# nvpro-samples/vk_gltf_renderer

Hardware: AMD Instinct MI355X
Metric: Msamples/s (and ms/frame @ fixed spp) 1080p & 4K, 1/2/4/8 MI355X (higher is better)
Workload: dtype f32

## Files before the change

vk_gltf_renderer_amd/csrc/device/mi_pt_api.hip:

```cpp
#include <hip/hip_runtime.h>

#include <algorithm>
#include <chrono>
#include <cstdlib>
#include <cmath>
#include <cstdio>
#include <cstring>
#include <memory>
#include <string>
#include <vector>

#include "mi_pt.h"
#include "bvh_refit.h"
#include "dev_buf.h"
#include "material_patch.h"
#include "pt_build.h"
#include "pt_bvh.h"
#include "pt_deform.h"
#include "pt_kernels.h"

namespace {

thread_local std::string g_lastError;

int fail(int code, const std::string& msg)
{
  g_lastError = msg;
  return code;
}

#define HIP_TRY(x)                                                                                                       \
  do                                                                                                                    \
  {                                                                                                                     \
    hipError_t e_ = (x);                                                                                                \
    if(e_ != hipSuccess)                                                                                                \
      return fail(MI_PT_ERR_HIP, std::string(#x) + ": " + hipGetErrorString(e_));                                       \
  } while(0)

using pt::DevBuf;

enum TimedKernel { TK_GENERATE, TK_TRACE, TK_SORT, TK_SHADE, TK_SHADOW, TK_ACCUM, TK_PRIMARY, TK_SHADE_FIRST, TK_COUNT };

}

struct RunSwitches
{
  int    packetInterval = 1;
  int    sortMode       = 2;
  bool   noPacket       = false;
  bool   stateBySlot    = false;
  bool   traceSpans     = false;
  int    overlapUpTo    = 32;
  int    overlapMinTris = 200000;
  bool   noPlanes       = false;
  bool   noOpaqueTris   = false;
  bool   noQuads        = false;
  bool   shadowFarFirst = true;
  int    reinsert       = 16;
  int    reinsertUpdate = 0;
  int    reinsertRounds = 4;
  float  splitFactor    = 4.0f;
  int    splitMaxDepth  = 8;
  float  splitMinShare  = 0.1f;
  bool   collapseGreedy = false;
  bool   collapseBad    = false;
  bool   hostCollapse   = false;
  bool   coreTex        = true;
  bool   shadowDeposit  = true;
  int    maxItersDiag   = 0;
  int    failBuildAt    = 0;
  bool   candPoolSet    = false;
  size_t candPool       = 0;
  void   read()
  {
    auto flag = [](const char* n) { const char* e = getenv(n); return e != nullptr; };
    auto num  = [](const char* n, int d) { const char* e = getenv(n); return e ? atoi(e) : d; };
    packetInterval = num("MI_PT_PACKET_INTERVAL", 1);
    sortMode       = num("MI_PT_SORT", 2);
    noPacket       = flag("MI_PT_NO_PACKET");
    stateBySlot    = flag("MI_PT_STATE_BY_SLOT");
    traceSpans     = flag("MI_PT_TRACE_SPANS");
    overlapUpTo    = num("MI_PT_OVERLAP", 32);
    overlapMinTris = num("MI_PT_OVERLAP_MIN_TRIS", 200000);
    noPlanes       = flag("MI_PT_DIAG_NO_PLANES");
    noOpaqueTris   = flag("MI_PT_DIAG_NO_OPAQUE_TRIS");
    noQuads        = flag("MI_PT_DIAG_NO_QUADS");
    shadowFarFirst = num("MI_PT_SHADOW_FAR_FIRST", 1) != 0;
    reinsert       = std::max(0, num("MI_PT_REINSERT", 16));
    reinsertUpdate = std::max(0, num("MI_PT_REINSERT_UPDATE", 0));
    reinsertRounds = std::max(1, num("MI_PT_REINSERT_ROUNDS", 4));
    if(const char* e = getenv("MI_PT_SPLIT"))
      splitFactor = std::max(0.0f, float(atof(e)));
    if(const char* e = getenv("MI_PT_SPLIT_MIN_SHARE"))
      splitMinShare = std::max(0.0f, float(atof(e)));
    splitMaxDepth  = std::min(std::max(0, num("MI_PT_SPLIT_DEPTH", 8)), 10);
    if(const char* e = getenv("MI_PT_COLLAPSE"))
    {
      collapseGreedy = strcmp(e, "greedy") == 0;
      collapseBad    = !collapseGreedy && strcmp(e, "sah") != 0;
    }
    hostCollapse   = flag("MI_PT_HOST_COLLAPSE");
    maxItersDiag   = num("MI_PT_DIAG_MAX_ITERS", 0);
    coreTex        = num("MI_PT_CORE_TEX", 1) != 0;
    shadowDeposit  = num("MI_PT_SHADOW_DEPOSIT", 1) != 0;
    failBuildAt    = num("MI_PT_DIAG_FAIL_BUILD", 0);
    if(const char* e = getenv("MI_PT_DIAG_CAND_POOL"))
    {
      candPoolSet = true;
      candPool    = size_t(strtoull(e, nullptr, 10));
    }
  }
};

struct MiPt
{
  int device = 0;
  int numCUs = 256;
  RunSwitches sw;
  int accelBuilds = 0;
  int               frameQueueDepth = 1;
  int               pendingFrames   = 0;
  MiPathtraceParams pendingFirst{};
  void*             pendingStream   = nullptr;
  DevBuf<MiGltfShadeMaterial> materials;
  DevBuf<MiGltfTextureInfo>   texInfos;
  DevBuf<pt::DevTexRef>       texRefs;
  DevBuf<pt::DevCoreTex>      coreTex;
  DevBuf<MiGltfRenderNode>    nodes;
  DevBuf<pt::DevPrim>         prims;
  DevBuf<MiGltfLight>         lights;
  DevBuf<pt::DevTexture>      textures;
  DevBuf<uchar4>              texels;
  DevBuf<uint4>               texQuads;
  DevBuf<uint8_t>             geometry;
  DevBuf<uint8_t>             instFlags;
  DevBuf<float>               srgbLut;
  DevBuf<float4>              envPixels;
// ... 176 lines not shown
    return rc;
  if(!vertexMotionActive(pt))
    return MI_PT_OK;
  const size_t numPrims = pt->hostPrims.size();
  pt->vmPrevOffset.assign(numPrims, SIZE_MAX);
  size_t                bytes = 0;
  std::vector<uint32_t> ids;
  for(int id : pt->deformPrimIDs)
  {
    pt->vmPrevOffset[size_t(id)] = bytes;
    bytes += align16(size_t(pt->primVertices[size_t(id)]) * 12);
    pt->vmMaxVertices = std::max(pt->vmMaxVertices, pt->primVertices[size_t(id)]);
    ids.push_back(uint32_t(id));
  }
  HIP_TRY(pt->vmPrevPositions.alloc(std::max<size_t>(bytes, 16)));
  std::vector<pt::VertexMotionPrim> table(numPrims);
  for(size_t i = 0; i < numPrims; ++i)
  {
    pt::VertexMotionPrim& v = table[i];
    v.prevPositions = pt->vmPrevOffset[i] != SIZE_MAX ? reinterpret_cast<const float*>(pt->vmPrevPositions.ptr + pt->vmPrevOffset[i]) : nullptr;
    v.positions     = pt->hostPrims[i].positions;
    v.indices       = pt->hostPrims[i].indices;
    v.numTriangles  = i < pt->primTriangles.size() ? pt->primTriangles[i] : 0u;
    v.vertexCount   = pt->primVertices[i];
  }
  HIP_TRY(pt->vmPrims.upload(table.data(), table.size()));
  HIP_TRY(pt->vmDeformIDs.upload(ids.data(), ids.size()));
  pt::launchSnapshotPositions(pt->vmPrims.ptr, pt->vmDeformIDs.ptr, uint32_t(ids.size()), pt->vmMaxVertices, nullptr);
  HIP_TRY(hipGetLastError());
  HIP_TRY(hipDeviceSynchronize());
  return MI_PT_OK;
}

int allocPathResources(MiPt* pt, int frames)
{
  if(size_t(pt->numSlots) * size_t(frames) >= 0x7fffffffull)
    return fail(MI_PT_ERR_ARGUMENT, "too many path slots: reduce the frames in flight or the resolution");
  pt->framesCap          = frames;
  const size_t n         = std::max(size_t(pt->numSlots) * size_t(frames), size_t(1));
  HIP_TRY(pt->pathArrays.alloc(n));
  HIP_TRY(pt->firstHit.alloc(std::max(size_t(pt->numSlots), size_t(1))));
  pt->haveFirstHit = false;
  pt->optThroughput.release(); pt->optMisc.release(); pt->optMedium.release(); pt->optPixelSum.release(); pt->optGuides.release(); pt->optShadowAux2.release();
  pt::PathSoA& P = pt->paths;
  P              = pt::PathSoA{};
  P.radiance     = pt->pathArrays.ptr;
  P.firstHit     = pt->firstHit.ptr;
  if(int rc = allocFirstHitTri(pt))
    return rc;
  const size_t numChunks = (n + pt::QCHUNK - 1) / pt::QCHUNK;
  const size_t subCap    = ((numChunks + pt::NSUB - 1) / pt::NSUB + 1) * pt::QCHUNK;
  const size_t qsize     = subCap * pt::NSUB;
  if(qsize >= (size_t(1) << 31))
    return fail(MI_PT_ERR_ARGUMENT, "mi_pt_render_frames: " + std::to_string(frames) + " frames in flight x " + std::to_string(pt->numSlots)
                                        + " pixel slots exceed 2^31 path slots");
  HIP_TRY(pt->queueMem.alloc(qsize * 3 + pt::QC_COUNT));
  HIP_TRY(pt->queuePayload.alloc(qsize * 14));
  pt->queueCap = qsize;
  pt::RayQueue* qs[3] = {&pt->queues.active[0], &pt->queues.active[1], &pt->queues.shadow};
  for(int i = 0; i < 3; ++i)
    qs[i]->slot = pt->queueMem.ptr + qsize * size_t(i);
  for(int i = 0; i < 2; ++i)
  {
    qs[i]->org  = pt->queuePayload.ptr + qsize * size_t(5 * i + 0);
    qs[i]->dir  = pt->queuePayload.ptr + qsize * size_t(5 * i + 1);
    qs[i]->aux2 = pt->queuePayload.ptr + qsize * size_t(5 * i + 2);
    qs[i]->misc = pt->queuePayload.ptr + qsize * size_t(5 * i + 3);
    qs[i]->rad  = pt->queuePayload.ptr + qsize * size_t(5 * i + 4);
    qs[i]->aux  = pt->queuePayload.ptr + qsize * 10;
  }
  pt->queues.shadow.org  = pt->queuePayload.ptr + qsize * 11;
  pt->queues.shadow.dir  = pt->queuePayload.ptr + qsize * 12;
  pt->queues.shadow.aux  = pt->queuePayload.ptr + qsize * 13;
  pt->queues.shadow.aux2 = nullptr;
  pt->queues.shadow.misc = pt->queues.shadow.rad = nullptr;
  pt->queues.counters = pt->queueMem.ptr + 3 * qsize;
  pt->queues.subCap   = uint32_t(subCap);
  pt->queues.candPool = nullptr; pt->queues.candNext = nullptr; pt->queues.overflow = nullptr;
  pt->queues.candCap  = 0;
  size_t candCap = qsize * 2;
  if(pt->sw.candPoolSet)
    candCap = pt->sw.candPool;
  if(pt->hasTransmissive && pt->wide && candCap > 0)
  {
// ... 765 lines not shown
  }
  {
    std::string why;
    if(!materialSlotsInRange(sd->materials, sd->numMaterials, sd->numTextureInfos, why))
      return fail(MI_PT_ERR_ARGUMENT, "mi_pt_create: " + why);
  }
  for(int i = 0; i < sd->numRenderPrimitives; ++i)
  {
    const MiPtRenderPrimitive& p = sd->renderPrimitives[i];
    if(p.vertexCount > 0 && !p.positions)
      return fail(MI_PT_ERR_ARGUMENT, "mi_pt_create: render primitive " + std::to_string(i) + " has vertices but no positions");
    if(p.triangleCount > 0 && !p.indices)
      return fail(MI_PT_ERR_ARGUMENT, "mi_pt_create: render primitive " + std::to_string(i) + " has triangles but no indices");
    for(size_t k = 0, n = size_t(p.triangleCount) * 3; k < n; ++k)
      if(p.indices[k] >= p.vertexCount)
        return fail(MI_PT_ERR_ARGUMENT, "mi_pt_create: render primitive " + std::to_string(i) + " has a vertex index beyond its vertexCount");
  }

  static const bool buildTiming = getenv("MI_PT_BUILD_TIMING") != nullptr;
  auto              tPhase      = std::chrono::steady_clock::now();
  auto              phase       = [&](const char* what) {
    if(!buildTiming)
      return;
    (void)hipDeviceSynchronize();
    const auto now = std::chrono::steady_clock::now();
    fprintf(stderr, "[mi_pt build] %-28s %8.2f ms\n", what, std::chrono::duration<double, std::milli>(now - tPhase).count());
    tPhase = now;
  };

  std::unique_ptr<MiPt> pt(new MiPt());
  pt->sw.read();
  if(pt->sw.collapseBad)
    return fail(MI_PT_ERR_ARGUMENT, std::string("MI_PT_COLLAPSE=") + getenv("MI_PT_COLLAPSE") + " is neither \"sah\" nor \"greedy\"");
  pt->device          = device;
  pt->numCUs          = prop.multiProcessorCount > 0 ? prop.multiProcessorCount : 256;
  pt->collectCounters = options && options->collectCounters;

  HIP_TRY(pt->materials.upload(sd->materials, size_t(sd->numMaterials)));
  HIP_TRY(pt->texInfos.upload(sd->textureInfos, size_t(sd->numTextureInfos)));
  HIP_TRY(pt->nodes.upload(sd->renderNodes, size_t(sd->numRenderNodes)));
  HIP_TRY(pt->lights.upload(sd->lights, size_t(sd->numLights)));

  size_t geomBytes = 0;
  for(int i = 0; i < sd->numRenderPrimitives; ++i)
  {
    const MiPtRenderPrimitive& p = sd->renderPrimitives[i];
    geomBytes += align16(size_t(p.triangleCount) * 12);
    geomBytes += align16(size_t(p.vertexCount) * 12);
    if(p.normals) geomBytes += align16(size_t(p.vertexCount) * 12);
    if(p.colors) geomBytes += align16(size_t(p.vertexCount) * 4);
    if(p.tangents) geomBytes += align16(size_t(p.vertexCount) * 16);
    if(p.texCoords0) geomBytes += align16(size_t(p.vertexCount) * 8);
    if(p.texCoords1) geomBytes += align16(size_t(p.vertexCount) * 8);
    geomBytes += align16(size_t(p.vertexCount) * 48);
  }
  if(geomBytes / 16 >= (size_t(1) << 32))
    return fail(MI_PT_ERR_ARGUMENT, "the geometry pool exceeds 64 GiB");
  HIP_TRY(pt->geometry.alloc(std::max<size_t>(geomBytes, 16)));
  std::vector<uint8_t>     staging(std::max<size_t>(geomBytes, 16));
  std::vector<pt::DevPrim> devPrims(size_t(sd->numRenderPrimitives));
  {
    size_t off = 0;
    auto   put = [&](const void* src, size_t bytes) -> const uint8_t* {
      if(!src || bytes == 0)
        return nullptr;
      memcpy(staging.data() + off, src, bytes);
// ... 772 lines not shown
  c.fc.numFrames = numFrames;
  pt::divideMagic(uint32_t(std::max(numFrames, 2)), c.fc.framesMagic, c.fc.framesShift);
  c.fc.slotLayout = numFrames % 64 == 0 ? 1 : 0;
  c.fc.stateInQueue = (!pt->sw.stateBySlot && !(pt->frameInfo.flags & MI_SCENE_INFINITE_PLANE_SHADOW_CATCHER)) ? 1 : 0;
  const bool guides = (params->flags & MI_PT_USE_OPTIX_DENOISER) != 0;
  if(int rc = ensureOptionalPathArrays(pt, c.fc.stateInQueue == 0, params->numSamples > 1, guides, (pt->frameInfo.flags & MI_SCENE_INFINITE_PLANE_SHADOW_CATCHER) != 0))
    return rc;
  c.paths        = pt->paths;
  {
    const bool stateBySlot = c.fc.stateInQueue == 0, multiSample = params->numSamples > 1;
    if(!(stateBySlot || multiSample))
      c.paths.misc = nullptr;
    if(!stateBySlot)
      c.paths.throughput = nullptr;
    if(!multiSample)
      c.paths.pixelSum = nullptr;
  }
  pt->accumFrames   = float(params->totalSamples) / float(params->numSamples) + float(numFrames);
  if(guides && (params->totalSamples == 0 || pt->momentFrames == pt->accumFrames - float(numFrames)))
    pt->momentFrames = pt->accumFrames;
  else if(!guides || params->totalSamples == 0)
    pt->momentFrames = 0.0f;
  if(!guides)
  {
    c.paths.guideAlbedo = nullptr;
    c.paths.guideNormal = nullptr;
  }
  c.queues           = pt->queues;
  if(!(pt->frameInfo.flags & MI_SCENE_INFINITE_PLANE_SHADOW_CATCHER))
    c.queues.shadow.aux2 = nullptr;
  c.ownedTiles       = pt->ownedTiles.ptr;
  c.stats            = pt->stats.ptr;
  c.stream           = stream;
  c.persistentBlocks = unsigned(pt->numCUs) * 8u;
  c.hasAlpha         = pt->hasAlpha;
  c.hasAlphaClosest  = c.hasAlpha && pt->hasAlphaTest;
  c.visualization    = pt->frameInfo.visualization > MI_VIZ_RENDERED && pt->frameInfo.visualization < MI_VIZ_COUNT;
  if(pt->frameInfo.visualization == MI_VIZ_OPACITY_MICROMAP)
    c.hasAlphaClosest = false;
  c.hasTransmissive  = pt->hasTransmissive;
  c.simpleMaterials  = pt->simpleMaterials;
  c.wide             = pt->wide;
  c.collectCounters  = pt->collectCounters;
  c.shadowDeposit    = pt->sw.shadowDeposit;
  {
    c.sortMode = pt->sw.sortMode;
  }
  if(pt->sceneDevDirty)
  {
    HIP_TRY(hipDeviceSynchronize());
    HIP_TRY(pt->sceneDev.upload(&pt->scene, 1));
    pt->sceneDevDirty = false;
  }
  if(!pt->fcHost)
  {
    HIP_TRY(hipHostMalloc(reinterpret_cast<void**>(&pt->fcHost), sizeof(pt::FrameConsts) * MiPt::FC_RING, hipHostMallocDefault));
    HIP_TRY(pt->fcRing.alloc(MiPt::FC_RING));
    for(hipEvent_t& e : pt->fcDone)
      HIP_TRY(hipEventCreateWithFlags(&e, hipEventDisableTiming));
  }
  const unsigned fcSlot = pt->fcCursor++ % unsigned(MiPt::FC_RING);
  if(pt->fcCursor > unsigned(MiPt::FC_RING))
    HIP_TRY(hipEventSynchronize(pt->fcDone[fcSlot]));
  pt->fcHost[fcSlot] = c.fc;
  HIP_TRY(hipMemcpyAsync(pt->fcRing.ptr + fcSlot, pt->fcHost + fcSlot, sizeof(pt::FrameConsts), hipMemcpyHostToDevice, stream));
  c.sceneDev = pt->sceneDev.ptr;
  c.fcDev    = pt->fcRing.ptr + fcSlot;

  auto timedOn = [&](hipStream_t on, int kind, auto&& launch) {
    if(pt->timingEnabled)
    {
      hipEvent_t a = getEvent(pt, pt->evCursor), b = getEvent(pt, pt->evCursor);
      (void)hipEventRecord(a, on);
      launch();
      (void)hipEventRecord(b, on);
      pt->pendingSpans.push_back({kind, a, b});
    }
// ... 709 lines not shown
```

vk_gltf_renderer_amd/csrc/device/pt_kernels.h:

```cpp
#pragma once
#include <hip/hip_runtime.h>

#include "pt_scene.h"
#include "pt_temporal.h"

namespace pt {

struct LaunchCtx
{
  DevScene        scene;
  FrameConsts     fc;
  const DevScene*    sceneDev;
  const FrameConsts* fcDev;
  PathSoA         paths;
  Queues          queues;
  const uint32_t* ownedTiles;
  StatCounters*   stats;
  hipStream_t     stream;
  unsigned        persistentBlocks;
  bool            hasAlpha;
  bool            hasAlphaClosest;
  bool            hasTransmissive;
  bool            simpleMaterials;
  bool            wide;
  bool            collectCounters;
  bool            shadowDeposit;
  int             sortMode;
  bool            visualization;
};

void launchBuildShadeRecords(const DevScene& scene, uint32_t numTris, DevShadeTri* out, hipStream_t s);
void launchBuildAlphaRecords(const DevScene& scene, uint32_t numTris, DevAlphaTri* out, hipStream_t s);
void launchPatchMaterials(const DevScene& scene, const uint8_t* instFlags, const uint8_t* dirty, DevTri* tris, DevAlphaTri* alphaTris, DevShadeTri* shadeTris,
                          uint32_t numTris, hipStream_t s);
void dumpTraceProfile();
void launchBvh8Planes(const uint4* nodes, uint32_t numNodes, float* planes, hipStream_t s);
void launchTextureQuads(const uchar4* texels, uint4* quads, uint32_t offset, int width, int height, int wrapS, int wrapT, hipStream_t s);
void launchResetCounters(const Queues& Q, hipStream_t s);
void launchSkyPrecomp(const MiSkyPhysicalParameters& sky, SkyPrecomp* out, hipStream_t stream);
void launchGenerate(const LaunchCtx& c, int sampleIndex);
void launchTraceClosest(const LaunchCtx& c, int cur);
void launchTracePrimary(const LaunchCtx& c, int sampleIndex);
void launchShade(const LaunchCtx& c, int cur, bool first);
void launchTraceShadow(const LaunchCtx& c, int nxt);
void launchFlushSurvivors(const LaunchCtx& c, int cur);
void launchFinishSample(const LaunchCtx& c, int sampleIndex, float4* accum, float* depth, float4* albedo, float4* normal);
void launchSelection(const LaunchCtx& c, uint32_t* selection);
void launchQueryRays(const DevScene& scene, bool wide, bool any, const MiPtRay* rays, uint32_t numRays, MiPtRayHit* hits, hipStream_t s);
void launchPickRays(const DevScene& scene, const FrameConsts& fc, bool wide, const float2* xy, uint32_t numRays, MiPtRayHit* hits, hipStream_t s);

void launchAtrous(const float4* in, float4* out, const float4* albedo, const float4* normal, int width, int height, int step, float sigmaColor,
                  float sigmaNormal, float sigmaAlbedo, hipStream_t s);

const float4* launchSvgf(const float4* color, const float4* albedo, const float4* normal, const float* depth, float4* bufA, float4* bufB, int width, int height,
                         int iterations, float frames, float sigmaLuminance, float sigmaNormal, float sigmaDepth, hipStream_t s);

const float4* launchSvgfFilter(float4* in, float4* other, const float4* color, const float4* albedo, const float4* normal, const float* depth, int width,
                               int height, int iterations, float sigmaLuminance, float sigmaNormal, float sigmaDepth, hipStream_t s);

// ... 13 lines not shown
```

vk_gltf_renderer_amd/csrc/device/pt_kernels.hip:

```cpp
#include <hip/hip_runtime.h>
#include <hip/hip_fp16.h>

#ifndef MI_PT_EXACT_FP
#define PT_FAST_SHADING_MATH 1
#endif
#include "pt_kernels.h"
#include "pt_shading.h"
#include "pt_bvh.h"
#include "pt_bvh8.h"
#include "pt_camera.h"
#include "pt_packet.h"
#include "pt_feed.h"
#include "pt_visualize.h"

namespace pt {

namespace {

constexpr int TRACE_BLOCK = 1024;
#ifndef NODE_CACHE_EXTRA
#define NODE_CACHE_EXTRA 0
#endif
constexpr int NODE_CACHE  = 712 + NODE_CACHE_EXTRA;
constexpr int NODE_CACHE_ALPHA = 504 + NODE_CACHE_EXTRA;
constexpr int SEL_BLOCK   = 256;
#ifndef TRACE_MIN_WAVES
#define TRACE_MIN_WAVES 1
#endif
constexpr int SHADE_BLOCK = 256;
constexpr uint32_t SORT_ROUNDS   = 4;
constexpr uint32_t SORT_WINDOW   = SORT_ROUNDS * SHADE_BLOCK;
constexpr uint32_t SORT_SEGMENTS = SORT_ROUNDS * (SHADE_BLOCK / 64);
constexpr int      SORT_BINS     = 32;
constexpr uint32_t SORT_BIN_MISS = 30;
constexpr uint32_t SORT_BIN_DEAD = 31;
#ifndef SHADE_SIMPLE_WAVES
#define SHADE_SIMPLE_WAVES 3
#endif

PT_DEV uint32_t laneId() { return __lane_id(); }

PT_DEV void queuePrefix(const uint32_t* counts, uint32_t* s_prefix)
{
  if(threadIdx.x < 64)
  {
// ... 33 lines not shown
    s_tmp[0] = 0;
    s_tmp[1] = 0;
  }
  __syncthreads();
  const unsigned long long maskN = __ballot(predNext), maskS = __ballot(predShadow);
  const uint32_t           lane  = laneId();
  uint32_t                 wbaseN = 0, wbaseS = 0;
  if(lane == 0)
  {
    if(maskN != 0ull)
      wbaseN = atomicAdd(&s_tmp[0], uint32_t(__popcll(maskN)));
    if(maskS != 0ull)
      wbaseS = atomicAdd(&s_tmp[1], uint32_t(__popcll(maskS)));
  }
  wbaseN = uint32_t(__shfl(int(wbaseN), 0));
  wbaseS = uint32_t(__shfl(int(wbaseS), 0));
  __syncthreads();
  if(threadIdx.x == 0)
  {
    const uint32_t     nN = s_tmp[0], nS = s_tmp[1];
    unsigned long long base = 0ull;
    if((nN | nS) != 0u)
      base = atomicAdd(reinterpret_cast<unsigned long long*>(pair), (static_cast<unsigned long long>(nS) << 32) | nN);
    s_tmp[2] = uint32_t(base);
    s_tmp[3] = uint32_t(base >> 32);
  }
  __syncthreads();
  const unsigned long long below = (1ull << lane) - 1ull;
  PushPos                  p;
  p.next   = sub * subCap + s_tmp[2] + wbaseN + uint32_t(__popcll(maskN & below));
  p.shadow = sub * subCap + s_tmp[3] + wbaseS + uint32_t(__popcll(maskS & below));
  return p;
}



PT_DEV bool slotToPixel(const FrameConsts& fc, const uint32_t* ownedTiles, uint32_t slot, int& px, int& py)
{
  const uint32_t tile  = ownedTiles[slot >> (2 * fc.tileShift)];
  const uint32_t w     = slot & ((1u << (2 * fc.tileShift)) - 1u);
  const uint32_t micro = w >> 6, lane = w & 63u;
  const uint32_t mshift = uint32_t(fc.tileShift) - 3u;
  px                   = int((tile & 0xffffu) + (micro & ((1u << mshift) - 1u)) * 8u + (lane & 7u));
  py                   = int((tile >> 16) + (micro >> mshift) * 8u + (lane >> 3));
  return px < fc.width && py < fc.height;
}


PT_DEV uint4 packMedium(f3 ext, f3 sc, float g)
{
  __half2 a = __floats2half2_rn(ext.x, ext.y), b = __floats2half2_rn(ext.z, sc.x), c = __floats2half2_rn(sc.y, sc.z), d = __floats2half2_rn(g, 0.0f);
  uint4   r;
  r.x = *reinterpret_cast<uint32_t*>(&a);
  r.y = *reinterpret_cast<uint32_t*>(&b);
  r.z = *reinterpret_cast<uint32_t*>(&c);
  r.w = *reinterpret_cast<uint32_t*>(&d);
  return r;
}
PT_DEV void unpackMedium(uint4 m, f3& ext, f3& sc, float& g)
{
  float2 a = __half22float2(*reinterpret_cast<__half2*>(&m.x)), b = __half22float2(*reinterpret_cast<__half2*>(&m.y));
  float2 c = __half22float2(*reinterpret_cast<__half2*>(&m.z)), d = __half22float2(*reinterpret_cast<__half2*>(&m.w));
  ext = mk3(a.x, a.y, b.x);
  sc  = mk3(b.y, c.x, c.y);
  g   = d.x;
}

struct CameraPath
// ... 1154 lines not shown
        if((G.bits >> 8) == 0u)
        {
          if(st2.sp == 0)
            break;
          G = st2.pop();
        }
        const uint32_t child = groupPopChild(G, octinv);
        if(G.bits >> 8)
          st2.push(G);
        uint32_t tBase, tMask;
        bvh8Visit(sc, r, bestT, octinv, child, G, tBase, tMask, nullptr, 0u);
        while(leafPending(tMask))
        {
          const int k = int(leafPop(tMask, 0u));
          testTri(int(tBase) + k);
        }
      }
    }
    else
    {
      LaneStack st;
      int       stackOverflow[BVH_STACK_PRIV];
      st.lds = s_stack; st.tid = int(threadIdx.x); st.stride = SEL_BLOCK; st.sp = 0; st.priv = stackOverflow;
      bvhWalk(sc, r, bestT, st, [&](int triIndex, float) -> float {
        testTri(triIndex);
        return bestT;
      });
    }
  }
  selection[size_t(py) * size_t(fc.width) + size_t(px)] = (bestRnode != 0xffffffffu) ? bestRnode + 1u : 0u;
}

template <bool COUNT, bool SIMPLE, bool FIRST>
__global__ void __launch_bounds__(SHADE_BLOCK, SIMPLE ? SHADE_SIMPLE_WAVES : 1) k_shade(const DevScene* __restrict__ scp, const FrameConsts* __restrict__ fcp, PathSoA P, Queues Q, int cur, int sortMode, StatCounters* stats)
{
  constexpr bool VIZ = false;
#include "pt_shade_body.h"
}
template <bool SIMPLE, bool FIRST>
__global__ void __launch_bounds__(SHADE_BLOCK, SIMPLE ? SHADE_SIMPLE_WAVES : 1) k_shade_viz(const DevScene* __restrict__ scp, const FrameConsts* __restrict__ fcp, PathSoA P, Queues Q, int cur, int sortMode, StatCounters* stats)
{
  constexpr bool COUNT = false, VIZ = true;
#include "pt_shade_body.h"
}

template <int MODE>
struct ShadowCfg
{
  static constexpr int BLOCK = MODE == 2 ? 256 : TRACE_BLOCK;
  static constexpr int CACHE = MODE == 2 ? 320 : (MODE == 1 ? NODE_CACHE_ALPHA : (MODE == 3 ? NODE_CACHE_ALPHA - 104 : NODE_CACHE));
};

PT_DEV void shadowDeposit(const PathSoA& P, const Queues& Q, int nxt, uint32_t slot, uint32_t qpos, bool catcherRay, f3 contrib, f3 total, bool occ,
                          float catcherDarken)
{
  if(!catcherRay)
  {
    if(!occ)
    {
      float4* const target = shadowTarget(P, Q, nxt, slot);
      float4        rad    = *target;
      rad.x += contrib.x * total.x;
      rad.y += contrib.y * total.y;
      rad.z += contrib.z * total.z;
      *target = rad;
    }
    return;
  }
  const float4 a2  = Q.shadow.aux2[qpos];
  const f3     sf  = occ ? mk3(0.0f) : total;
  float4       rad = P.radiance[slot];
  if(sf.x == 1.0f && sf.y == 1.0f && sf.z == 1.0f)
  {
// ... 939 lines not shown
  dim3           grid(batchSlots / 256u), block(256);
  const bool interval = c.fc.slotLayout == 1 && c.scene.packetInterval != 0 && c.scene.bvh8Planes != nullptr;
#define MI_LAUNCH_PRIMARY(A, C)                                                                                                                   \
  do                                                                                                                                              \
  {                                                                                                                                               \
    if(interval)                                                                                                                                  \
      hipLaunchKernelGGL((k_trace_primary<A, C, true>), grid, block, 0, c.stream, c.scene, c.fc, c.sceneDev, c.fcDev, c.paths, c.queues, c.ownedTiles, sampleIndex, batchSlots, c.stats);  \
    else                                                                                                                                          \
      hipLaunchKernelGGL((k_trace_primary<A, C, false>), grid, block, 0, c.stream, c.scene, c.fc, c.sceneDev, c.fcDev, c.paths, c.queues, c.ownedTiles, sampleIndex, batchSlots, c.stats); \
  } while(0)
  if(c.hasAlphaClosest)
  {
    if(c.collectCounters) MI_LAUNCH_PRIMARY(true, true); else MI_LAUNCH_PRIMARY(true, false);
  }
  else
  {
    if(c.collectCounters) MI_LAUNCH_PRIMARY(false, true); else MI_LAUNCH_PRIMARY(false, false);
  }
#undef MI_LAUNCH_PRIMARY
}
void launchTraceClosest(const LaunchCtx& c, int cur)
{
  if(c.wide)
    launchTraceClosestT<true>(c, cur);
  else
    launchTraceClosestT<false>(c, cur);
}
void launchShade(const LaunchCtx& c, int cur, bool first)
{
  dim3 grid(c.persistentBlocks), block(SHADE_BLOCK);
  if(c.visualization)
  {
#define MI_LAUNCH_SHADE_VIZ(S, F) \
  hipLaunchKernelGGL((k_shade_viz<S, F>), grid, block, 0, c.stream, c.sceneDev, c.fcDev, c.paths, c.queues, cur, (S ? 0 : c.sortMode), c.stats)
    if(c.simpleMaterials)
    {
      if(first) MI_LAUNCH_SHADE_VIZ(true, true); else MI_LAUNCH_SHADE_VIZ(true, false);
    }
    else
    {
      if(first) MI_LAUNCH_SHADE_VIZ(false, true); else MI_LAUNCH_SHADE_VIZ(false, false);
    }
#undef MI_LAUNCH_SHADE_VIZ
    return;
  }
#define MI_LAUNCH_SHADE(C, S, F) \
  hipLaunchKernelGGL((k_shade<C, S, F>), grid, block, 0, c.stream, c.sceneDev, c.fcDev, c.paths, c.queues, cur, (S ? 0 : c.sortMode), c.stats)
#define MI_LAUNCH_SHADE_F(C, S) do { if(first) MI_LAUNCH_SHADE(C, S, true); else MI_LAUNCH_SHADE(C, S, false); } while(0)
  if(c.simpleMaterials)
  {
    if(c.collectCounters) MI_LAUNCH_SHADE_F(true, true); else MI_LAUNCH_SHADE_F(false, true);
  }
  else
  {
    if(c.collectCounters) MI_LAUNCH_SHADE_F(true, false); else MI_LAUNCH_SHADE_F(false, false);
  }
#undef MI_LAUNCH_SHADE_F
#undef MI_LAUNCH_SHADE
}
void launchTraceShadow(const LaunchCtx& c, int nxt)
{
  if(c.wide)
    launchTraceShadowT<true>(c, nxt);
  else
    launchTraceShadowT<false>(c, nxt);
}
void launchFlushSurvivors(const LaunchCtx& c, int cur)
{
  hipLaunchKernelGGL(k_flush_survivors, dim3(c.persistentBlocks), dim3(256), 0, c.stream, c.paths, c.queues, cur);
}
void launchFinishSample(const LaunchCtx& c, int sampleIndex, float4* accum, float* depth, float4* albedo, float4* normal)
{
  unsigned grid = (unsigned(c.fc.numSlots) + 255u) / 256u;
  hipLaunchKernelGGL(k_finish_sample, dim3(grid), dim3(256), 0, c.stream, c.fc, c.sceneDev, c.fcDev, c.paths, c.ownedTiles, sampleIndex, accum, depth, albedo, normal);
}
void launchSelection(const LaunchCtx& c, uint32_t* selection)
{
  unsigned grid = (unsigned(c.fc.numSlots) + SEL_BLOCK - 1) / SEL_BLOCK;
  if(c.wide)
    hipLaunchKernelGGL(k_selection<true>, dim3(grid), dim3(SEL_BLOCK), 0, c.stream, c.scene, c.fc, c.ownedTiles, selection);
// ... 6 lines not shown
```

vk_gltf_renderer_amd/csrc/device/pt_shade_body.h:

```cpp
  const DevScene&    sc = uniformConst(*scp);
  const FrameConsts& fc = uniformConst(*fcp);
  const bool         stateInQueue = fc.stateInQueue != 0;
  __shared__ uint32_t s_prefix[NSUB + 1];
  __shared__ uint32_t s_push[4];
  __shared__ float    s_srgb[256];
#ifndef SHADE_NO_DEFERRED_MISS
  constexpr bool DEFER_MISS = !FIRST;
#else
  constexpr bool DEFER_MISS = false;
#endif
  __shared__ uint32_t s_missPos[DEFER_MISS ? 2 * SHADE_BLOCK : 1];
  __shared__ uint32_t s_missCount;
  const bool          deferMiss = DEFER_MISS && !hasFlag(fc.frameInfo.flags, MI_SCENE_USE_INFINITE_PLANE) && !hasFlag(fc.frameInfo.flags, MI_SCENE_USE_HDR_ENVIRONMENT);
  if(threadIdx.x == 0)
    s_missCount = 0;
  auto finishMisses = [&](bool all) {
    __syncthreads();
    const uint32_t n = s_missCount;
    if(n == 0u || (!all && n < uint32_t(SHADE_BLOCK)))
      return;
    const uint32_t take = min(n, uint32_t(SHADE_BLOCK)), base = n - take;
    uint32_t       pos = 0;
    if(threadIdx.x < take)
      pos = s_missPos[base + threadIdx.x];
    __syncthreads();
    if(threadIdx.x == 0)
      s_missCount = base;
    if(threadIdx.x < take)
    {
      const uint32_t slot  = Q.active[cur].slot[pos];
      const float4   d4    = Q.active[cur].dir[pos];
      const float4   misc4 = stateInQueue ? Q.active[cur].misc[pos] : P.misc[slot];
      const float4   tp4   = stateInQueue ? Q.active[cur].aux2[pos] : P.throughput[slot];
      const float4   rad4  = stateInQueue ? Q.active[cur].rad[pos] : P.radiance[slot];
      f3             radiance = xyz(rad4);
      f3             envColor;
      float          mis;
      missEnvironment(sc, fc, xyz(d4), tp4.w, envColor, mis);
      radiance += xyz(tp4) * mis * envColor;
      uint32_t flags = __float_as_uint(misc4.y) & (PF_INSIDE | PF_NOT_SOLID | (0xffu << PF_DEPTH_SHIFT) | (0xffu << PF_SCATTER_SHIFT));
      if(SIMPLE)
        flags &= ~uint32_t(PF_INSIDE);
      const bool solid = !(flags & PF_NOT_SOLID);
      P.radiance[slot] = make_float4(radiance.x, radiance.y, radiance.z, __uint_as_float(__float_as_uint(fmaxf(fabsf(rad4.w), 0.0f)) | (solid ? 0u : RADW_NOT_SOLID)));
      if(P.misc)
        P.misc[slot] = make_float4(misc4.x, __uint_as_float(flags), misc4.z, misc4.w);
    }
    __syncthreads();
  };
  constexpr bool CAN_SORT = !SIMPLE;
  __shared__ uint32_t s_order[CAN_SORT ? SORT_WINDOW : 1];
  __shared__ uint16_t s_segCount[CAN_SORT ? SORT_SEGMENTS : 1][SORT_BINS];
  __shared__ uint32_t s_binBase[SORT_BINS + 1];
  static_assert(SHADE_BLOCK == 256, "one table entry per thread");
  if(blockIdx.x == 0 && threadIdx.x < 8)
  {
    Q.counters[QC_HEADS_TRACE + threadIdx.x] = 0;
    Q.counters[QC_HEADS_SHADOW + threadIdx.x]   = 0;
    Q.counters[QC_HEADS_OVERFLOW + threadIdx.x] = 0;
    if(threadIdx.x == 0)
      Q.counters[QC_CAND_POOL] = Q.counters[QC_RESOLVE] = Q.counters[QC_OVERFLOW] = 0;
  }
  queuePrefix(&Q.counters[cur ? QC_PAIR1 : QC_PAIR0], s_prefix);
  const uint32_t count      = s_prefix[NSUB];
  const int      nxt        = cur ^ 1;
  constexpr uint32_t ROUNDS = CAN_SORT ? SORT_ROUNDS : 1u;
  constexpr uint32_t WINDOW = ROUNDS * SHADE_BLOCK;
  const uint32_t     numWindows = (count + WINDOW - 1) / WINDOW;
  if(blockIdx.x >= numWindows)
    return;
  s_srgb[threadIdx.x] = sc.srgbLut[threadIdx.x];
  __syncthreads();
  const uint32_t wave = threadIdx.x >> 6, lane = threadIdx.x & 63u;
  for(uint32_t win = blockIdx.x; win < numWindows; win += gridDim.x)
  {
    uint32_t live = min(WINDOW, count - win * WINDOW);
    if(CAN_SORT && sortMode != 0)
    {
    uint32_t myPos[SORT_ROUNDS], myBin[SORT_ROUNDS], myRank[SORT_ROUNDS];
    for(uint32_t t = threadIdx.x; t < SORT_SEGMENTS * SORT_BINS; t += SHADE_BLOCK)
      (&s_segCount[0][0])[t] = 0;
    __syncthreads();
#pragma unroll
    for(uint32_t k = 0; k < SORT_ROUNDS; ++k)
    {
      const uint32_t i = win * WINDOW + k * SHADE_BLOCK + threadIdx.x;
      uint32_t       bin = SORT_BIN_DEAD;
      myPos[k]           = 0u;
      if(i < count)
      {
        myPos[k]            = queuePos(Q.subCap, s_prefix, i);
        const uint32_t slot = Q.active[cur].slot[myPos[k]];
        if(slot != QUEUE_DEAD)
        {
          const int tri = __float_as_int(Q.active[cur].aux[myPos[k]].y);
          if(tri < 0)
            bin = SORT_BIN_MISS;
          else
            bin = sortMode >= 2 ? uint32_t(sc.shadeTris[tri].materialID) % SORT_BIN_MISS : 0u;
        }
      }
      myBin[k] = bin;
      uint32_t           rank = 0;
      unsigned long long todo = __ballot(bin != SORT_BIN_DEAD);
      while(todo != 0ull)
      {
// ... 107 lines not shown
                          mk3(1.0f - hit4.z - hit4.w, hit4.z, hit4.w), rn.worldToObject, rn.objectToWorld, rayDir, VIZ ? &frontFace : nullptr);
        if(P.firstHitTri && firstRay && needFirstHit)
          P.firstHitTri[pathSlotPixel(fc, slot)] = make_uint4(uint32_t(S.renderPrimID), S.prim, __float_as_uint(hit4.z), __float_as_uint(hit4.w));
        if constexpr(VIZ)
        {
          rprimID = S.renderPrimID;
          if(fc.frameInfo.visualization == MI_VIZ_OPACITY_MICROMAP)
            ommState = (__float_as_uint(gat(sc.tris, triIdx).c.w) & INST_FORCE_OPAQUE) ? 0 : 1;
        }
      }
      else
        hitT = INFINITE_F;
      SPROF_END(0);

      bool hitInfinitePlane = false;
      {
        const float t = infinitePlaneT(fc, rayOrigin, rayDir, hitT);
        if(t > 0.0f)
        {
          hitT             = t;
          hit.pos          = rayOrigin + rayDir * hitT;
          hit.shadowPos    = hit.pos;
          hit.nrm          = mk3(0, 1, 0);
          hit.geonrm       = mk3(0, 1, 0);
          hit.tangent      = mk3(1, 0, 0);
          hit.bitangent    = mk3(0, 0, 1);
          hitInfinitePlane = true;
        }
      }

      if(deferMiss && hitT == INFINITE_F && !firstRay)
      {
        SPROF_BEGIN();
        s_missPos[atomicAdd(&s_missCount, 1u)] = inPos;
        deferred = true;
        done     = true;
        SPROF_END(6);
      }
      else if(hitT == INFINITE_F)
      {
        SPROF_BEGIN();
        bool backplate = false;
        if(firstRay)
        {
          solid             = false;
          if(needFirstHit)
            P.firstHit[pathSlotPixel(fc, slot)] = make_float4(rayDir.x, rayDir.y, rayDir.z, 0.0f);
          backplate = primaryMissBackplate(sc, fc, rayDir, radiance);
        }
        if(!backplate)
        {
          f3    envColor;
          float mis;
          missEnvironment(sc, fc, rayDir, lastSamplePdf, envColor, mis);
          radiance += throughput * mis * envColor;
        }
        done = true;
        SPROF_END(6);
      }

      if(!done)
      {
        PbrMaterial pbrMat;
        float worldFoot = (coneWidth + fc.pc.pixelAngle * hitT) / fmaxf(fabsf(dot(hit.geonrm, -rayDir)), 1e-3f);
        bool  unlit     = false;
        bool  catcherPlane = false;
        if(hitInfinitePlane)
// ... 247 lines not shown

      if(FIRST && P.guideAlbedo && !guideWritten && fc.pc.numSamples == 1)
      {
        P.guideAlbedo[slot] = make_float4(0, 0, 0, 0);
        P.guideNormal[slot] = make_float4(0, 0, 0, 0);
      }
      alive = !done && surfaceDepth < maxDepth;
      flags = (isInside ? PF_INSIDE : 0u) | (solid ? 0u : PF_NOT_SOLID) | (alive ? PF_ALIVE : 0u) | (uint32_t(min(surfaceDepth, 255)) << PF_DEPTH_SHIFT)
              | (uint32_t(scatterBounces) << PF_SCATTER_SHIFT);
      nextRad  = make_float4(radiance.x, radiance.y, radiance.z, __uint_as_float(__float_as_uint(fmaxf(maxRoughness.x, 0.0f)) | (solid ? 0u : RADW_NOT_SOLID)));
      nextMisc = make_float4(maxRoughness.y, __uint_as_float(flags), __uint_as_float(seed), coneWidth);
      if((!stateInQueue || !alive) && !deferred)
      {
        P.radiance[slot] = nextRad;
        if(P.misc)
          P.misc[slot] = nextMisc;
      }
      if(alive)
      {
        nextOrg = make_float4(rayOrigin.x, rayOrigin.y, rayOrigin.z, 0.0f);
        nextDir = make_float4(rayDir.x, rayDir.y, rayDir.z, __uint_as_float(seed));
        nextThr = make_float4(throughput.x, throughput.y, throughput.z, lastSamplePdf);
        if(!stateInQueue)
          P.throughput[slot] = nextThr;
      }
      if(COUNT && taps)
        atomicAdd(&stats->textureTaps, (unsigned long long)taps);
      if(COUNT && (meshHit || hitInfinitePlane))
        atomicAdd(&stats->surfaceHits, 1ull);
    }
#ifdef SHADE_PROFILE
    const unsigned long long sprofPush0 = __builtin_amdgcn_s_memtime();
#endif
    const PushPos  pp      = queuePushBlock2(alive, pushShadow, Q.subCap, &Q.counters[(nxt ? QC_PAIR1 : QC_PAIR0) + 2 * (chunk % NSUB)], chunk % NSUB, s_push);
    const uint32_t posNext = pp.next, posShadow = pp.shadow;
    if(alive)
    {
      Q.active[nxt].slot[posNext] = slot;
      Q.active[nxt].org[posNext]  = nextOrg;
      Q.active[nxt].dir[posNext]  = nextDir;
      if(stateInQueue)
      {
        Q.active[nxt].rad[posNext]  = nextRad;
        Q.active[nxt].misc[posNext] = nextMisc;
        Q.active[nxt].aux2[posNext] = nextThr;
      }
    }
    if(pushShadow)
    {
      Q.shadow.slot[posShadow] = (stateInQueue && alive) ? (posNext | SHADOW_TARGET_QUEUE) : slot;
      Q.shadow.org[posShadow]  = shOrg;
      Q.shadow.dir[posShadow]  = shDir;
      Q.shadow.aux[posShadow]  = shCon;
      if(catcher)
        Q.shadow.aux2[posShadow] = make_float4(shCon2.x, shCon2.y, shCon2.z, __uint_as_float(alive ? posNext : 0xffffffffu));
    }
#ifdef SHADE_PROFILE
    if(!FIRST && laneId() == 0)
    {
      const unsigned long long t_ = __builtin_amdgcn_s_memtime();
      atomicAdd(&g_shadeProf[14], t_ - sprofPush0);
      atomicAdd(&g_shadeProf[15], (t_ - sprofPush0) * (unsigned long long)__popcll(__ballot(alive || pushShadow)));
    }
    const unsigned long long sprofFin0 = __builtin_amdgcn_s_memtime();
#endif
    if(DEFER_MISS && deferMiss)
      finishMisses(false);
#ifdef SHADE_PROFILE
    if(!FIRST && laneId() == 0)
    {
      const unsigned long long t_ = __builtin_amdgcn_s_memtime();
      atomicAdd(&g_shadeProf[16], t_ - sprofFin0);
      atomicAdd(&g_shadeProf[18], t_ - sprofRound0);
      atomicAdd(&g_shadeProf[19], (t_ - sprofRound0) * (unsigned long long)__popcll(__ballot(inRange && slot != QUEUE_DEAD)));
    }
#endif
   }
   if(CAN_SORT)
     __syncthreads();
  }
  if(DEFER_MISS && deferMiss)
  {
    finishMisses(true);
    finishMisses(true);
  }
```

Baseline: 755.8.

## Use per-wave chunked queue appends and wave-local miss deferral in simple shade

In the simple-material shade kernel, block-wide queue pushes are replaced by per-wave appends. Each wave reserves chunks of queue slots with one 64-bit atomic and pads unused slots with dead markers. Deferred-miss handling moves from block-level __syncthreads to per-wave lists using wave barriers. Together these aim to cut block synchronisation and atomic contention. In exchange, queue capacity grows to hold slack, and downstream consumers must skip dead slots left in the queues.

```diff
diff --git a/vk_gltf_renderer_amd/csrc/device/mi_pt_api.hip b/vk_gltf_renderer_amd/csrc/device/mi_pt_api.hip
--- a/vk_gltf_renderer_amd/csrc/device/mi_pt_api.hip
+++ b/vk_gltf_renderer_amd/csrc/device/mi_pt_api.hip
@@ -18,6 +18,7 @@
 #include "pt_bvh.h"
 #include "pt_deform.h"
 #include "pt_kernels.h"
+#include "pt_append.h"
 
 namespace {
 
@@ -67,6 +68,9 @@
   bool   hostCollapse   = false;
   bool   coreTex        = true;
   bool   shadowDeposit  = true;
+  bool   shadeAppendBlock = false;
+  bool   shadeAppendBad   = false;
+  int    shadePieceDiag   = 0;
   int    maxItersDiag   = 0;
   int    failBuildAt    = 0;
   bool   candPoolSet    = false;
@@ -103,6 +107,12 @@
     maxItersDiag   = num("MI_PT_DIAG_MAX_ITERS", 0);
     coreTex        = num("MI_PT_CORE_TEX", 1) != 0;
     shadowDeposit  = num("MI_PT_SHADOW_DEPOSIT", 1) != 0;
+    if(const char* e = getenv("MI_PT_SHADE_APPEND"))
+    {
+      shadeAppendBlock = strcmp(e, "block") == 0;
+      shadeAppendBad   = !shadeAppendBlock && strcmp(e, "wave") != 0;
+    }
+    shadePieceDiag = std::max(0, num("MI_PT_DIAG_SHADE_PIECE", 0));
     failBuildAt    = num("MI_PT_DIAG_FAIL_BUILD", 0);
     if(const char* e = getenv("MI_PT_DIAG_CAND_POOL"))
     {
@@ -345,6 +355,8 @@
   return MI_PT_OK;
 }
 
+unsigned persistentBlocks(const MiPt* pt) { return unsigned(pt->numCUs) * 8u; }
+
 int allocPathResources(MiPt* pt, int frames)
 {
   if(size_t(pt->numSlots) * size_t(frames) >= 0x7fffffffull)
@@ -362,7 +374,8 @@
   if(int rc = allocFirstHitTri(pt))
     return rc;
   const size_t numChunks = (n + pt::QCHUNK - 1) / pt::QCHUNK;
-  const size_t subCap    = ((numChunks + pt::NSUB - 1) / pt::NSUB + 1) * pt::QCHUNK;
+  const size_t waveSlack = pt::appendSlack(persistentBlocks(pt), pt::APPEND_WAVES_PER_BLOCK, pt::NSUB, pt::APPEND_CHUNK_CAP);
+  const size_t subCap    = ((numChunks + pt::NSUB - 1) / pt::NSUB + 1 + (waveSlack + pt::QCHUNK - 1) / pt::QCHUNK) * pt::QCHUNK;
   const size_t qsize     = subCap * pt::NSUB;
   if(qsize >= (size_t(1) << 31))
     return fail(MI_PT_ERR_ARGUMENT, "mi_pt_render_frames: " + std::to_string(frames) + " frames in flight x " + std::to_string(pt->numSlots)
@@ -1194,6 +1207,8 @@
   pt->sw.read();
   if(pt->sw.collapseBad)
     return fail(MI_PT_ERR_ARGUMENT, std::string("MI_PT_COLLAPSE=") + getenv("MI_PT_COLLAPSE") + " is neither \"sah\" nor \"greedy\"");
+  if(pt->sw.shadeAppendBad)
+    return fail(MI_PT_ERR_ARGUMENT, std::string("MI_PT_SHADE_APPEND=") + getenv("MI_PT_SHADE_APPEND") + " is neither \"wave\" nor \"block\"");
   pt->device          = device;
   pt->numCUs          = prop.multiProcessorCount > 0 ? prop.multiProcessorCount : 256;
   pt->collectCounters = options && options->collectCounters;
@@ -2032,7 +2047,7 @@
   c.ownedTiles       = pt->ownedTiles.ptr;
   c.stats            = pt->stats.ptr;
   c.stream           = stream;
-  c.persistentBlocks = unsigned(pt->numCUs) * 8u;
+  c.persistentBlocks = persistentBlocks(pt);
   c.hasAlpha         = pt->hasAlpha;
   c.hasAlphaClosest  = c.hasAlpha && pt->hasAlphaTest;
   c.visualization    = pt->frameInfo.visualization > MI_VIZ_RENDERED && pt->frameInfo.visualization < MI_VIZ_COUNT;
@@ -2043,6 +2058,7 @@
   c.wide             = pt->wide;
   c.collectCounters  = pt->collectCounters;
   c.shadowDeposit    = pt->sw.shadowDeposit;
+  c.shadeAppendMode  = pt->sw.shadeAppendBlock ? 1 : (pt->sw.shadePieceDiag >= 64 ? pt->sw.shadePieceDiag : 0);
   {
     c.sortMode = pt->sw.sortMode;
   }
diff --git a/vk_gltf_renderer_amd/csrc/device/pt_append.h b/vk_gltf_renderer_amd/csrc/device/pt_append.h
--- /dev/null
+++ b/vk_gltf_renderer_amd/csrc/device/pt_append.h
@@ -0,0 +1,90 @@
+#pragma once
+#include <hip/hip_runtime.h>
+#include <cstdint>
+
+#ifndef PT_DEV
+#define PT_DEV __device__ __forceinline__
+#endif
+
+namespace pt {
+
+#ifndef APPEND_CHUNK_CAP_N
+#define APPEND_CHUNK_CAP_N 256
+#endif
+constexpr uint32_t APPEND_CHUNK_CAP   = APPEND_CHUNK_CAP_N;
+constexpr uint32_t APPEND_EXACT_BELOW = 16u * 64u;
+constexpr uint32_t APPEND_WAVES_PER_BLOCK = 4u;
+
+struct AppendRange
+{
+  uint32_t cur, end;
+};
+struct AppendTake
+{
+  uint32_t cur, rem, fresh;
+};
+
+PT_DEV uint32_t appendChunk(uint32_t inputCount, uint32_t grid, uint32_t wavesPerBlock, uint32_t nsub, uint32_t cap, uint32_t forced = 0u)
+{
+  if(grid % nsub != 0u)
+    return 0u;
+  if(forced >= 64u)
+    return (forced < cap ? forced : cap) & ~63u;
+  const uint32_t waves   = grid * wavesPerBlock;
+  const uint32_t perWave = waves ? inputCount / waves : 0u;
+  if(perWave < APPEND_EXACT_BELOW)
+    return 0u;
+  uint32_t c = (perWave / 16u) & ~63u;
+  if(c > cap)
+    c = cap;
+  return c & ~63u;
+}
+PT_DEV uint32_t appendWant(const AppendRange& r, uint32_t need, uint32_t chunk)
+{
+  const uint32_t rem = r.end - r.cur;
+  if(need <= rem)
+    return 0u;
+  return chunk != 0u ? chunk : need - rem;
+}
+PT_DEV AppendTake appendAdvance(AppendRange& r, uint32_t need, uint32_t want, uint32_t base)
+{
+  const AppendTake t{r.cur, r.end - r.cur, base};
+  if(want != 0u)
+  {
+    r.cur = base + (need - t.rem);
+    r.end = base + want;
+  }
+  else
+    r.cur += need;
+  return t;
+}
+PT_DEV uint32_t appendPos(const AppendTake& t, uint32_t rank) { return rank < t.rem ? t.cur + rank : t.fresh + (rank - t.rem); }
+
+struct WaveAppend
+{
+  AppendRange next, shadow;
+  uint32_t    sub;
+};
+struct AppendTakes
+{
+  AppendTake next, shadow;
+};
+template <class FetchAdd>
+PT_DEV AppendTakes appendRound(WaveAppend& a, uint32_t nNext, uint32_t nShadow, uint32_t chunk, FetchAdd&& fetchAdd)
+{
+  const uint32_t     wantN = appendWant(a.next, nNext, chunk), wantS = appendWant(a.shadow, nShadow, chunk);
+  unsigned long long base = 0ull;
+  if((wantN | wantS) != 0u)
+    base = fetchAdd((static_cast<unsigned long long>(wantS) << 32) | wantN);
+  AppendTakes t;
+  t.next   = appendAdvance(a.next, nNext, wantN, uint32_t(base));
+  t.shadow = appendAdvance(a.shadow, nShadow, wantS, uint32_t(base >> 32));
+  return t;
+}
+
+inline uint32_t appendSlack(uint32_t grid, uint32_t wavesPerBlock, uint32_t nsub, uint32_t cap)
+{
+  return ((grid + nsub - 1u) / nsub) * wavesPerBlock * (cap - 1u);
+}
+
+}
diff --git a/vk_gltf_renderer_amd/csrc/device/pt_kernels.h b/vk_gltf_renderer_amd/csrc/device/pt_kernels.h
--- a/vk_gltf_renderer_amd/csrc/device/pt_kernels.h
+++ b/vk_gltf_renderer_amd/csrc/device/pt_kernels.h
@@ -25,6 +25,7 @@
   bool            wide;
   bool            collectCounters;
   bool            shadowDeposit;
+  int             shadeAppendMode;
   int             sortMode;
   bool            visualization;
 };
diff --git a/vk_gltf_renderer_amd/csrc/device/pt_kernels.hip b/vk_gltf_renderer_amd/csrc/device/pt_kernels.hip
--- a/vk_gltf_renderer_amd/csrc/device/pt_kernels.hip
+++ b/vk_gltf_renderer_amd/csrc/device/pt_kernels.hip
@@ -11,6 +11,7 @@
 #include "pt_camera.h"
 #include "pt_packet.h"
 #include "pt_feed.h"
+#include "pt_append.h"
 #include "pt_visualize.h"
 
 namespace pt {
@@ -110,8 +111,35 @@
   p.shadow = sub * subCap + s_tmp[3] + wbaseS + uint32_t(__popcll(maskS & below));
   return p;
 }
-
-
+__device__ __noinline__ PushPos queuePushBlock2Call(bool predNext, bool predShadow, uint32_t subCap, uint32_t* pair, uint32_t sub)
+{
+  __shared__ uint32_t s_tmp[4];
+  return queuePushBlock2(predNext, predShadow, subCap, pair, sub, s_tmp);
+}
+
+static_assert(SHADE_BLOCK / 64 == int(APPEND_WAVES_PER_BLOCK), "appendSlack sizes the queues for this many waves per block");
+PT_DEV PushPos queuePushWave2(WaveAppend& a, bool predNext, bool predShadow, uint32_t chunk, uint32_t subCap, uint32_t* pair)
+{
+  const unsigned long long maskN = __ballot(predNext), maskS = __ballot(predShadow);
+  const AppendTakes        t     = appendRound(a, uint32_t(__popcll(maskN)), uint32_t(__popcll(maskS)), chunk, [&](unsigned long long add) {
+    unsigned long long base = 0ull;
+    if(laneId() == 0)
+      base = atomicAdd(reinterpret_cast<unsigned long long*>(pair), add);
+    const uint32_t lo = __builtin_amdgcn_readfirstlane(uint32_t(base)), hi = __builtin_amdgcn_readfirstlane(uint32_t(base >> 32));
+    return (static_cast<unsigned long long>(hi) << 32) | lo;
+  });
+  const unsigned long long below = (1ull << laneId()) - 1ull;
+  PushPos                  p;
+  p.next   = a.sub * subCap + appendPos(t.next, uint32_t(__popcll(maskN & below)));
+  p.shadow = a.sub * subCap + appendPos(t.shadow, uint32_t(__popcll(maskS & below)));
+  return p;
+}
+PT_DEV void appendMarkDead(uint32_t* slots, AppendRange& r)
+{
+  for(uint32_t p = r.cur + laneId(); p < r.end; p += 64u)
+    slots[p] = QUEUE_DEAD;
+  r.cur = r.end;
+}
 
 PT_DEV bool slotToPixel(const FrameConsts& fc, const uint32_t* ownedTiles, uint32_t slot, int& px, int& py)
 {
@@ -1332,13 +1360,13 @@
 }
 
 template <bool COUNT, bool SIMPLE, bool FIRST>
-__global__ void __launch_bounds__(SHADE_BLOCK, SIMPLE ? SHADE_SIMPLE_WAVES : 1) k_shade(const DevScene* __restrict__ scp, const FrameConsts* __restrict__ fcp, PathSoA P, Queues Q, int cur, int sortMode, StatCounters* stats)
+__global__ void __launch_bounds__(SHADE_BLOCK, SIMPLE ? SHADE_SIMPLE_WAVES : 1) k_shade(const DevScene* __restrict__ scp, const FrameConsts* __restrict__ fcp, PathSoA P, Queues Q, int cur, int sortMode, int appendMode, StatCounters* stats)
 {
   constexpr bool VIZ = false;
 #include "pt_shade_body.h"
 }
 template <bool SIMPLE, bool FIRST>
-__global__ void __launch_bounds__(SHADE_BLOCK, SIMPLE ? SHADE_SIMPLE_WAVES : 1) k_shade_viz(const DevScene* __restrict__ scp, const FrameConsts* __restrict__ fcp, PathSoA P, Queues Q, int cur, int sortMode, StatCounters* stats)
+__global__ void __launch_bounds__(SHADE_BLOCK, SIMPLE ? SHADE_SIMPLE_WAVES : 1) k_shade_viz(const DevScene* __restrict__ scp, const FrameConsts* __restrict__ fcp, PathSoA P, Queues Q, int cur, int sortMode, int appendMode, StatCounters* stats)
 {
   constexpr bool COUNT = false, VIZ = true;
 #include "pt_shade_body.h"
@@ -2344,7 +2372,7 @@
   if(c.visualization)
   {
 #define MI_LAUNCH_SHADE_VIZ(S, F) \
-  hipLaunchKernelGGL((k_shade_viz<S, F>), grid, block, 0, c.stream, c.sceneDev, c.fcDev, c.paths, c.queues, cur, (S ? 0 : c.sortMode), c.stats)
+  hipLaunchKernelGGL((k_shade_viz<S, F>), grid, block, 0, c.stream, c.sceneDev, c.fcDev, c.paths, c.queues, cur, (S ? 0 : c.sortMode), c.shadeAppendMode, c.stats)
     if(c.simpleMaterials)
     {
       if(first) MI_LAUNCH_SHADE_VIZ(true, true); else MI_LAUNCH_SHADE_VIZ(true, false);
@@ -2357,7 +2385,7 @@
     return;
   }
 #define MI_LAUNCH_SHADE(C, S, F) \
-  hipLaunchKernelGGL((k_shade<C, S, F>), grid, block, 0, c.stream, c.sceneDev, c.fcDev, c.paths, c.queues, cur, (S ? 0 : c.sortMode), c.stats)
+  hipLaunchKernelGGL((k_shade<C, S, F>), grid, block, 0, c.stream, c.sceneDev, c.fcDev, c.paths, c.queues, cur, (S ? 0 : c.sortMode), c.shadeAppendMode, c.stats)
 #define MI_LAUNCH_SHADE_F(C, S) do { if(first) MI_LAUNCH_SHADE(C, S, true); else MI_LAUNCH_SHADE(C, S, false); } while(0)
   if(c.simpleMaterials)
   {
diff --git a/vk_gltf_renderer_amd/csrc/device/pt_shade_body.h b/vk_gltf_renderer_amd/csrc/device/pt_shade_body.h
--- a/vk_gltf_renderer_amd/csrc/device/pt_shade_body.h
+++ b/vk_gltf_renderer_amd/csrc/device/pt_shade_body.h
@@ -10,23 +10,43 @@
   constexpr bool DEFER_MISS = false;
 #endif
   __shared__ uint32_t s_missPos[DEFER_MISS ? 2 * SHADE_BLOCK : 1];
-  __shared__ uint32_t s_missCount;
+  constexpr bool     WAVE_MISS  = SIMPLE;
+  constexpr uint32_t MISS_GROUP = WAVE_MISS ? 64u : uint32_t(SHADE_BLOCK);
+  __shared__ uint32_t s_missCount[SHADE_BLOCK / 64];
+  __shared__ uint32_t s_missSeen;
+  const uint32_t      missList = WAVE_MISS ? (threadIdx.x >> 6) : 0u, missLane = WAVE_MISS ? (threadIdx.x & 63u) : threadIdx.x;
+  uint32_t* const     missPos  = s_missPos + (DEFER_MISS ? missList * 2u * MISS_GROUP : 0u);
   const bool          deferMiss = DEFER_MISS && !hasFlag(fc.frameInfo.flags, MI_SCENE_USE_INFINITE_PLANE) && !hasFlag(fc.frameInfo.flags, MI_SCENE_USE_HDR_ENVIRONMENT);
-  if(threadIdx.x == 0)
-    s_missCount = 0;
+  if(threadIdx.x < SHADE_BLOCK / 64)
+    s_missCount[threadIdx.x] = 0;
   auto finishMisses = [&](bool all) {
-    __syncthreads();
-    const uint32_t n = s_missCount;
-    if(n == 0u || (!all && n < uint32_t(SHADE_BLOCK)))
+    uint32_t n;
+    if(WAVE_MISS)
+    {
+      __builtin_amdgcn_wave_barrier();
+      n = __builtin_amdgcn_readfirstlane(s_missCount[missList]);
+    }
+    else
+    {
+      __syncthreads();
+      if(threadIdx.x == 0)
+        s_missSeen = s_missCount[0];
+      __syncthreads();
+      n = s_missSeen;
+    }
+    if(n == 0u || (!all && n < MISS_GROUP))
       return;
-    const uint32_t take = min(n, uint32_t(SHADE_BLOCK)), base = n - take;
+    const uint32_t take = min(n, MISS_GROUP), base = n - take;
     uint32_t       pos = 0;
-    if(threadIdx.x < take)
-      pos = s_missPos[base + threadIdx.x];
-    __syncthreads();
-    if(threadIdx.x == 0)
-      s_missCount = base;
-    if(threadIdx.x < take)
+    if(missLane < take)
+      pos = missPos[base + missLane];
+    if(WAVE_MISS)
+      __builtin_amdgcn_wave_barrier();
+    else
+      __syncthreads();
+    if(missLane == 0)
+      s_missCount[missList] = base;
+    if(missLane < take)
     {
       const uint32_t slot  = Q.active[cur].slot[pos];
       const float4   d4    = Q.active[cur].dir[pos];
@@ -46,7 +66,10 @@
       if(P.misc)
         P.misc[slot] = make_float4(misc4.x, __uint_as_float(flags), misc4.z, misc4.w);
     }
-    __syncthreads();
+    if(WAVE_MISS)
+      __builtin_amdgcn_wave_barrier();
+    else
+      __syncthreads();
   };
   constexpr bool CAN_SORT = !SIMPLE;
   __shared__ uint32_t s_order[CAN_SORT ? SORT_WINDOW : 1];
@@ -72,6 +95,9 @@
   s_srgb[threadIdx.x] = sc.srgbLut[threadIdx.x];
   __syncthreads();
   const uint32_t wave = threadIdx.x >> 6, lane = threadIdx.x & 63u;
+  const bool     waveAppend  = SIMPLE && appendMode != 1;
+  const uint32_t appendPiece = SIMPLE ? __builtin_amdgcn_readfirstlane(appendChunk(count, gridDim.x, APPEND_WAVES_PER_BLOCK, uint32_t(NSUB), APPEND_CHUNK_CAP, uint32_t(appendMode))) : 0u;
+  WaveAppend     wa{{0u, 0u}, {0u, 0u}, blockIdx.x % NSUB};
   for(uint32_t win = blockIdx.x; win < numWindows; win += gridDim.x)
   {
     uint32_t live = min(WINDOW, count - win * WINDOW);
@@ -245,7 +271,7 @@
       if(deferMiss && hitT == INFINITE_F && !firstRay)
       {
         SPROF_BEGIN();
-        s_missPos[atomicAdd(&s_missCount, 1u)] = inPos;
+        missPos[atomicAdd(&s_missCount[missList], 1u)] = inPos;
         deferred = true;
         done     = true;
         SPROF_END(6);
@@ -559,7 +585,22 @@
 #ifdef SHADE_PROFILE
     const unsigned long long sprofPush0 = __builtin_amdgcn_s_memtime();
 #endif
-    const PushPos  pp      = queuePushBlock2(alive, pushShadow, Q.subCap, &Q.counters[(nxt ? QC_PAIR1 : QC_PAIR0) + 2 * (chunk % NSUB)], chunk % NSUB, s_push);
+    uint32_t* const pair = &Q.counters[(nxt ? QC_PAIR1 : QC_PAIR0) + 2 * (chunk % NSUB)];
+    PushPos         pp;
+    if(!SIMPLE)
+      pp = queuePushBlock2(alive, pushShadow, Q.subCap, pair, chunk % NSUB, s_push);
+    else if(waveAppend)
+    {
+      if(wa.sub != chunk % NSUB)
+      {
+        appendMarkDead(Q.active[nxt].slot + wa.sub * Q.subCap, wa.next);
+        appendMarkDead(Q.shadow.slot + wa.sub * Q.subCap, wa.shadow);
+        wa.sub = chunk % NSUB;
+      }
+      pp = queuePushWave2(wa, alive, pushShadow, appendPiece, Q.subCap, pair);
+    }
+    else
+      pp = queuePushBlock2Call(alive, pushShadow, Q.subCap, pair, chunk % NSUB);
     const uint32_t posNext = pp.next, posShadow = pp.shadow;
     if(alive)
     {
@@ -606,6 +647,11 @@
    if(CAN_SORT)
      __syncthreads();
   }
+  if(SIMPLE)
+  {
+    appendMarkDead(Q.active[nxt].slot + wa.sub * Q.subCap, wa.next);
+    appendMarkDead(Q.shadow.slot + wa.sub * Q.subCap, wa.shadow);
+  }
   if(DEFER_MISS && deferMiss)
   {
     finishMisses(true);
```

New measurement: 755.1. About the same (-0.1%).
